# arihantb2/direct_lidar_odometry

Hardware: NVIDIA B200
Metric: scan_pairs_per_s (higher is better)
Workload: dtype f32 kNN / f64 GICP

## Files before the change

### direct_lidar_odometry_b200/csrc/knn_cov.cu

```cuda
#include <cstdio>
#include <cstdlib>
#include <mutex>
#include "internal.h"
#include "grid_search.cuh"
#include "gicp_math.cuh"
#include "sort_networks.inc"

namespace ngicp {

constexpr int KC_THREADS = 256;
constexpr int KC_WARPS = KC_THREADS / 32;
#ifndef KNN_MIN_BLOCKS
#define KNN_MIN_BLOCKS 5
#endif

__global__ void __launch_bounds__(KC_THREADS) knn_query_kernel(GridView g, const float4* __restrict__ queries, int nq, int k,
                                                               int* __restrict__ idx, float* __restrict__ d2) {
  const int lane = threadIdx.x & 31;
  const int warp = (blockIdx.x * blockDim.x + threadIdx.x) >> 5;
  const int nwarps = (gridDim.x * blockDim.x) >> 5;
  const GridParams gp = load_grid(g.desc);
  for (int q = warp; q < nq; q += nwarps) {
    const float4 qp = queries[q];
    WarpTopK rs;
// ... 6 lines not shown
      idx[(size_t)q * k + lane] = o;
      d2[(size_t)q * k + lane] = dd;
    }
  }
}

__global__ void __launch_bounds__(KC_THREADS, KNN_MIN_BLOCKS) knn_lists_kernel(GridView g, int n, int k, int* __restrict__ nbr, int q_lo, int q_hi) {
  const int lane = threadIdx.x & 31;
  const int warp = (blockIdx.x * blockDim.x + threadIdx.x) >> 5;
  const int nwarps = (gridDim.x * blockDim.x) >> 5;
  const GridParams gp = load_grid(g.desc);
  for (int q = q_lo + warp; q < q_hi; q += nwarps) {
    const float4 qp = __ldg(g.sorted + q);
    WarpTopK rs;
    rs.init(k, lane);
    if (isfinite(qp.x) && isfinite(qp.y) && isfinite(qp.z)) grid_search_warp(g, gp, qp.x, qp.y, qp.z, FLT_MAX, rs, k >= 4);
    if (lane < k) nbr[(size_t)q * k + lane] = rs.p;
  }
}

__global__ void __launch_bounds__(KC_THREADS) knn_query_wide_kernel(GridView g, const float4* __restrict__ queries, int nq, int k,
                                                                    int* __restrict__ idx, float* __restrict__ d2) {
  __shared__ float s_d[KC_WARPS][KNN_WIDE_MAX_K];
  __shared__ int s_p[KC_WARPS][KNN_WIDE_MAX_K];
  const int lane = threadIdx.x & 31, wib = threadIdx.x >> 5;
  const int warp = (blockIdx.x * blockDim.x + threadIdx.x) >> 5;
  const int nwarps = (gridDim.x * blockDim.x) >> 5;
  const GridParams gp = load_grid(g.desc);
  for (int q = warp; q < nq; q += nwarps) {
    const float4 qp = queries[q];
    WarpTopKWide rs;
    rs.init(k, lane, s_d[wib], s_p[wib]);
    if (isfinite(qp.x) && isfinite(qp.y) && isfinite(qp.z)) grid_search_warp(g, gp, qp.x, qp.y, qp.z, FLT_MAX, rs);
    __syncwarp();
    for (int j = lane; j < k; j += 32) {
      const int p = s_p[wib][j];
      idx[(size_t)q * k + j] = p >= 0 ? __float_as_int(__ldg(g.sorted + p).w) : -1;
      d2[(size_t)q * k + j] = p >= 0 ? s_d[wib][j] : -1.f;
    }
  }
}
__global__ void __launch_bounds__(KC_THREADS) knn_lists_wide_kernel(GridView g, int n, int k, int* __restrict__ nbr, int q_lo, int q_hi) {
  __shared__ float s_d[KC_WARPS][KNN_WIDE_MAX_K];
  __shared__ int s_p[KC_WARPS][KNN_WIDE_MAX_K];
  const int lane = threadIdx.x & 31, wib = threadIdx.x >> 5;
  const int warp = (blockIdx.x * blockDim.x + threadIdx.x) >> 5;
  const int nwarps = (gridDim.x * blockDim.x) >> 5;
  const GridParams gp = load_grid(g.desc);
  for (int q = q_lo + warp; q < q_hi; q += nwarps) {
    const float4 qp = __ldg(g.sorted + q);
    WarpTopKWide rs;
    rs.init(k, lane, s_d[wib], s_p[wib]);
    if (isfinite(qp.x) && isfinite(qp.y) && isfinite(qp.z)) grid_search_warp<WarpTopKWide, false, 4>(g, gp, qp.x, qp.y, qp.z, FLT_MAX, rs, true);
    __syncwarp();
    for (int j = lane; j < k; j += 32) nbr[(size_t)q * k + j] = s_p[wib][j];
  }
}

#ifndef TQ_WARPS
#define TQ_WARPS 2
#endif
#define TQ_POS_BITS 9
#define TQ_POS_MASK 0x1ffu
#ifndef TQ_CMAX
#define TQ_CMAX 448
#endif
#ifndef TQ_LCAP
#define TQ_LCAP 40
#endif
#ifndef TQ_CORE
#define TQ_CORE KNN_BRICK
#endif
#ifndef TQ_PACKED
#define TQ_PACKED 1
#endif
#ifndef TQ_UNROLL
#define TQ_UNROLL 1
#endif
#define NG_PRAGMA_(x) _Pragma(#x)
#define NG_UNROLL(n) NG_PRAGMA_(unroll n)
#ifndef TQ_SMAX
#define TQ_SMAX 16
#endif
constexpr int TQ_ITEM = 64;
struct TileSmem {
  float xs[TQ_CMAX], ys[TQ_CMAX], zs[TQ_CMAX];
  int slot[TQ_CMAX];
  unsigned lst[TQ_LCAP + 1][32];
  int cur[TQ_ITEM];
  float cur_t[TQ_ITEM];
  float cur_lo[TQ_ITEM], cur_hi[TQ_ITEM];
  int nxt[TQ_ITEM];
  int rowoff[68];
};

__device__ __forceinline__ float box_face_distance(const GridParams& gp, int x0, int x1, int y0, int y1, int z0, int z1,
                                                   float qx, float qy, float qz) {
  float m = FLT_MAX;
  if (x0 > 0) m = fminf(m, qx - (gp.ox + (float)x0 * gp.cell));
  if (x1 + 1 < gp.dx) m = fminf(m, (gp.ox + (float)(x1 + 1) * gp.cell) - qx);
  if (y0 > 0) m = fminf(m, qy - (gp.oy + (float)y0 * gp.cell));
  if (y1 + 1 < gp.dy) m = fminf(m, (gp.oy + (float)(y1 + 1) * gp.cell) - qy);
  if (z0 > 0) m = fminf(m, qz - (gp.oz + (float)z0 * gp.cell));
  if (z1 + 1 < gp.dz) m = fminf(m, (gp.oz + (float)(z1 + 1) * gp.cell) - qz);
  return m == FLT_MAX ? FLT_MAX : m - gp.margin;
}

#ifdef TQ_DEBUG
#define TQ_CHECK(cond, what, a, b) do { if (!(cond)) { printf("TQ_CHECK %s failed: %d %d (block %d thread %d)\n", what, (int)(a), (int)(b), blockIdx.x, threadIdx.x); __trap(); } } while (0)
#else
#define TQ_CHECK(cond, what, a, b) do { } while (0)
#endif
enum { ST_FALLBACK = 0, ST_TIES, ST_TILES, ST_PASSES, ST_LANES, ST_ITEMS, ST_DEC1, ST_DEC2, ST_DECHI, ST_PASS1, ST_PASS2, ST_PASSHI, ST_CAND, ST_TSUM, ST_TEND, ST_TSTART, ST_TWARPS, ST_N };
enum { CT_ITEMS = 0, CT_NEXT, CT_REST, CT_REST_NEXT, CT_DONE, CT_FIX, CT_SLOW, CT_N = 8 };

__device__ __forceinline__ void fb_append(unsigned mask, int slot, int lane, int* __restrict__ fb_list, int* __restrict__ fb_count,
                                          unsigned char* __restrict__ fb_flags) {
  if (!mask) return;
  if ((mask >> lane) & 1u) fb_flags[slot] = 1;
  const int leader = __ffs(mask) - 1;
  int base = 0;
  if (lane == leader) base = atomicAdd(fb_count, __popc(mask));
  base = __shfl_sync(FULL, base, leader);
  if ((mask >> lane) & 1u) fb_list[base + __popc(mask & ((1u << lane) - 1u))] = slot;
}

__device__ __forceinline__ void fix_append(unsigned mask, int slot, int lane, int n, int* __restrict__ fb_list, int* __restrict__ fix_count,
                                           unsigned char* __restrict__ fb_flags) {
  if (!mask) return;
  if ((mask >> lane) & 1u) fb_flags[slot] = 1;
  const int leader = __ffs(mask) - 1;
  int base = 0;
  if (lane == leader) base = atomicAdd(fix_count, __popc(mask));
  base = __shfl_sync(FULL, base, leader);
  if ((mask >> lane) & 1u) fb_list[n - 1 - (base + __popc(mask & ((1u << lane) - 1u)))] = slot;
}

__device__ __forceinline__ int warp_incl_scan(int v, int lane) {
#pragma unroll
  for (int o = 1; o < 32; o <<= 1) { const int t = __shfl_up_sync(FULL, v, o); if (lane >= o) v += t; }
  return v;
}
__device__ __forceinline__ int run_of(int inc, int t) {
  int j = 0;
#pragma unroll
  for (int step = 16; step > 0; step >>= 1) {
    const int v = __shfl_sync(FULL, inc, j + step - 1);
    if (v <= t) j += step;
  }
  return j;
}

__device__ __forceinline__ int box_population(const GridView& g, const GridParams& gp, int x0, int y0, int z0, int sz, int s, int sub, int nsub) {
  const int ny = sz + 2 * s, nrows = ny * ny;
  const int xl = max(x0 - s, 0), xr = min(x0 + sz - 1 + s, gp.dx - 1) + 1;
  int c = 0;
  for (int r = sub; r < nrows; r += nsub) {
    const int y = y0 - s + (r % ny), z = z0 - s + (r / ny);
    if (y >= 0 && y < gp.dy && z >= 0 && z < gp.dz && xl < xr) {
      const int* row = g.cell_start + (z * gp.dy + y) * gp.dx;
      c += __ldg(row + xr) - __ldg(row + xl);
    }
  }
  for (int o = nsub >> 1; o > 0; o >>= 1) c += __shfl_xor_sync(FULL, c, o);
  return c;
}

#ifndef TQ_BIG
#define TQ_BIG 32
#endif
__device__ __forceinline__ void emit_items(bool emit, bool slow, int x0, int y0, int z0, int sz, int q, int lane, int n, int4* __restrict__ items,
                                           int* __restrict__ ctrl) {
  const int nit = emit ? (q + TQ_ITEM - 1) / TQ_ITEM : 0;
  const int nfront = (slow || nit == 0 || q - (nit - 1) * TQ_ITEM > TQ_BIG) ? nit : nit - 1;
  const int nback = nit - nfront;
  if (__any_sync(FULL, nfront > 0)) {
    const int inc = warp_incl_scan(nfront, lane);
    const int total = __shfl_sync(FULL, inc, 31);
    int base = 0;
    if (lane == 0) base = atomicAdd(ctrl + CT_SLOW, total);
    base = __shfl_sync(FULL, base, 0) + inc - nfront;
    for (int i = 0; i < nfront; ++i) items[base + i] = make_int4(x0, y0, z0, sz | (i << 8));
  }
  const unsigned bm = __ballot_sync(FULL, nback > 0);
  if (bm) {
    int base = 0;
    if (lane == 0) base = atomicAdd(ctrl + CT_ITEMS, __popc(bm));
    base = __shfl_sync(FULL, base, 0) + __popc(bm & ((1u << lane) - 1u));
    if (nback > 0) items[n - 1 - base] = make_int4(x0, y0, z0, sz | ((nit - 1) << 8));
  }
}

__global__ void __launch_bounds__(256) brick_clear_kernel(GridView g, unsigned char* __restrict__ flags, long long flag_cap) {
  const GridParams gp = load_grid(g.desc);
  const long long nb = (long long)((gp.dx + TQ_CORE - 1) / TQ_CORE) * ((gp.dy + TQ_CORE - 1) / TQ_CORE) * ((gp.dz + TQ_CORE - 1) / TQ_CORE);
  if (nb > flag_cap) return;
// ... 11 lines not shown
  const int nbx = (gp.dx + TQ_CORE - 1) / TQ_CORE, nby = (gp.dy + TQ_CORE - 1) / TQ_CORE, nbz = (gp.dz + TQ_CORE - 1) / TQ_CORE;
  if ((long long)nbx * nby * nbz > flag_cap) return;
  for (int i = blockIdx.x * blockDim.x + threadIdx.x; i < n; i += gridDim.x * blockDim.x) {
    const float4 p = __ldg(g.sorted + i);
    const int bx = cell_coord(p.x, gp.ox, gp.inv, gp.dx) / TQ_CORE, by = cell_coord(p.y, gp.oy, gp.inv, gp.dy) / TQ_CORE,
              bz = cell_coord(p.z, gp.oz, gp.inv, gp.dz) / TQ_CORE;
    flags[((long long)bz * nby + by) * nbx + bx] = 1;
  }
}

#ifndef TQ_SLOW_FACTOR
#define TQ_SLOW_FACTOR 2
#endif
__global__ void __launch_bounds__(256) knn_plan_kernel(GridView g, int n, int k, int4* __restrict__ items, int* __restrict__ ctrl,
                                                       const unsigned char* __restrict__ flags, long long flag_cap) {
  const int lane = threadIdx.x & 31;
  const int nwarps = (gridDim.x * blockDim.x) >> 5;
  const GridParams gp = load_grid(g.desc);
  const int nbx = (gp.dx + TQ_CORE - 1) / TQ_CORE, nby = (gp.dy + TQ_CORE - 1) / TQ_CORE, nbz = (gp.dz + TQ_CORE - 1) / TQ_CORE;
  const int run = ((long long)nbx * nby * nbz > 32768) ? 8 : 1;
  const int nrx = (nbx + run - 1) / run;
  const int nruns = nrx * nby * nbz;
  for (int w = (blockIdx.x * blockDim.x + threadIdx.x) >> 5; w < nruns; w += nwarps) {
    const int rbx = (w % nrx) * run, rby = (w / nrx) % nby, rbz = w / (nrx * nby);
    unsigned occ = FULL;
    if (run > 1 && (long long)nbx * nby * nbz <= flag_cap) {
      int e = 0;
      if (lane < run && rbx + lane < nbx) e = flags[((long long)rbz * nby + rby) * nbx + rbx + lane];
      occ = __ballot_sync(FULL, e != 0);
      if (occ == 0u) continue;
    } else if (run > 1) {
      int e = 0;
      if (lane < TQ_CORE * TQ_CORE) {
        const int y = rby * TQ_CORE + (lane % TQ_CORE), z = rbz * TQ_CORE + (lane / TQ_CORE);
        if (y < gp.dy && z < gp.dz) {
          const int* row = g.cell_start + (z * gp.dy + y) * gp.dx;
          e = __ldg(row + min((rbx + run) * TQ_CORE, gp.dx)) - __ldg(row + rbx * TQ_CORE);
        }
      }
      if (!__any_sync(FULL, e != 0)) continue;
    }
    const int y0 = rby * TQ_CORE, z0 = rbz * TQ_CORE;
    unsigned deep_boxes;
    {
      const int bi = lane >> 2, sub = lane & 3;
      const bool valid = bi < run && rbx + bi < nbx && ((occ >> bi) & 1u);
      const int bx0 = valid ? (rbx + bi) * TQ_CORE : -(1 << 20);
      const int Qb = box_population(g, gp, bx0, y0, z0, TQ_CORE, 0, sub, 4);
      const int Cb = box_population(g, gp, Qb > 0 ? bx0 : -(1 << 20), y0, z0, TQ_CORE, 1, sub, 4);
      const bool fits = Qb > 0 && Cb <= TQ_CMAX;
      emit_items(sub == 0 && fits, Cb < TQ_SLOW_FACTOR * k, bx0, y0, z0, TQ_CORE, Qb, lane, n, items, ctrl);
      deep_boxes = __ballot_sync(FULL, sub == 0 && Qb > 0 && !fits);
    }
    for (; deep_boxes; deep_boxes &= deep_boxes - 1) {
      const int bi = (__ffs(deep_boxes) - 1) >> 2;
      const int x0 = (rbx + bi) * TQ_CORE;
      const int h = TQ_CORE / 2;
      const int ch = lane >> 2, sub = lane & 3;
      const int cx0 = x0 + (ch & 1) * h, cy0 = y0 + ((ch >> 1) & 1) * h, cz0 = z0 + (ch >> 2) * h;
      const int Qc = box_population(g, gp, cx0, cy0, cz0, h, 0, sub, 4);
      const int Cc = box_population(g, gp, cx0, cy0, cz0, h, 1, sub, 4);
      const bool fits = Cc <= TQ_CMAX;
      emit_items(sub == 0 && Qc > 0 && fits, false, cx0, cy0, cz0, h, Qc, lane, n, items, ctrl);
      unsigned deep = __ballot_sync(FULL, sub == 0 && Qc > 0 && !fits);
      for (; deep; deep &= deep - 1) {
        const int l = __ffs(deep) - 1;
        const int px = __shfl_sync(FULL, cx0, l), py = __shfl_sync(FULL, cy0, l), pz = __shfl_sync(FULL, cz0, l);
        const int gx = px + (ch & 1), gy = py + ((ch >> 1) & 1), gz = pz + (ch >> 2);
        const int Qg = box_population(g, gp, gx, gy, gz, 1, 0, sub, 4);
        emit_items(sub == 0 && Qg > 0, false, gx, gy, gz, 1, Qg, lane, n, items, ctrl);
      }
    }
  }
}

#ifndef TQ_TARGET_EXTRA
#define TQ_TARGET_EXTRA 14
#endif
__device__ __forceinline__ float lattice_floor(float t) { return __uint_as_float(__float_as_uint(t) & ~TQ_POS_MASK); }
struct Shrunk { float T2; int cnt; };
#ifndef TQ_SHRINK_F
#define TQ_SHRINK_F 0.75f
#endif
#ifndef TQ_COOP_SHRINK
#define TQ_COOP_SHRINK 1
#endif
#if TQ_COOP_SHRINK
__device__ __noinline__ Shrunk shrink_lists(TileSmem& S, unsigned om, float T2, int cnt) {
  const int lane = threadIdx.x & 31;
  const unsigned lt = (1u << lane) - 1u;
  Shrunk r;
  r.T2 = T2; r.cnt = cnt;
  for (; om; om &= om - 1) {
    const int L = __ffs(om) - 1;
    float t = __shfl_sync(FULL, T2, L);
    int n = __shfl_sync(FULL, cnt, L);
    do {
      t = lattice_floor(t * TQ_SHRINK_F);
      const unsigned tb = __float_as_uint(t);
      const unsigned e0 = lane < n ? S.lst[lane][L] : 0xffffffffu;
      const unsigned e1 = lane + 32 < n ? S.lst[lane + 32][L] : 0xffffffffu;
      const bool k0 = e0 < tb, k1 = e1 < tb;
      const unsigned m0 = __ballot_sync(FULL, k0), m1 = __ballot_sync(FULL, k1);
      __syncwarp();
      if (k0) S.lst[__popc(m0 & lt)][L] = e0;
      if (k1) S.lst[__popc(m0) + __popc(m1 & lt)][L] = e1;
      __syncwarp();
      n = __popc(m0) + __popc(m1);
    } while (n > TQ_LCAP - 4);
    if (lane == L) { r.T2 = t; r.cnt = n; }
  }
  return r;
}
#else
__device__ __noinline__ Shrunk shrink_list(unsigned* col, float T2, int cnt) {
  do {
    T2 = lattice_floor(T2 * 0.75f);
    const unsigned tb = __float_as_uint(T2);
    int pos = 0;
    for (int i = 0; i < cnt; ++i) {
      const unsigned e = col[i * 32];
      if (e < tb) { col[pos * 32] = e; ++pos; }
    }
    cnt = pos;
  } while (cnt > TQ_LCAP - 4);
  Shrunk r;
  r.T2 = T2; r.cnt = cnt;
  return r;
}
#endif
__device__ __forceinline__ unsigned long long f2_pack(float lo, float hi) { unsigned long long r; asm("mov.b64 %0, {%1, %2};" : "=l"(r) : "f"(lo), "f"(hi)); return r; }
__device__ __forceinline__ void f2_unpack(unsigned long long v, float& lo, float& hi) { asm("mov.b64 {%0, %1}, %2;" : "=f"(lo), "=f"(hi) : "l"(v)); }
__device__ __forceinline__ unsigned long long f2_sub(unsigned long long a, unsigned long long b) { unsigned long long r; asm("sub.rn.f32x2 %0, %1, %2;" : "=l"(r) : "l"(a), "l"(b)); return r; }
__device__ __forceinline__ unsigned long long f2_mul(unsigned long long a, unsigned long long b) { unsigned long long r; asm("mul.rn.f32x2 %0, %1, %2;" : "=l"(r) : "l"(a), "l"(b)); return r; }
__device__ __forceinline__ unsigned long long f2_fma(unsigned long long a, unsigned long long b, unsigned long long c) { unsigned long long r; asm("fma.rn.f32x2 %0, %1, %2, %3;" : "=l"(r) : "l"(a), "l"(b), "l"(c)); return r; }
struct Query2 { unsigned long long x, y, z, one; };
__device__ __forceinline__ unsigned long long sqdist2_unfused(const Query2& q, unsigned long long px, unsigned long long py, unsigned long long pz) {
#if TQ_PACKED
  const unsigned long long dx = f2_sub(q.x, px), dy = f2_sub(q.y, py), dz = f2_sub(q.z, pz);
  return f2_fma(f2_fma(f2_mul(dx, dx), q.one, f2_mul(dy, dy)), q.one, f2_mul(dz, dz));
#else
  float qx, qy, qz, t, x0, x1, y0, y1, z0, z1;
  f2_unpack(q.x, qx, t); f2_unpack(q.y, qy, t); f2_unpack(q.z, qz, t);
  f2_unpack(px, x0, x1); f2_unpack(py, y0, y1); f2_unpack(pz, z0, z1);
  return f2_pack(sqdist_unfused(qx, qy, qz, x0, y0, z0), sqdist_unfused(qx, qy, qz, x1, y1, z1));
#endif
}

__device__ __forceinline__ int collect_pass(TileSmem& S, unsigned* const col, int c, int cend, float qx, float qy, float qz, float one, float& T2_io, int cnt) {
  float T2 = T2_io;
  Query2 q;
  q.x = f2_pack(qx, qx); q.y = f2_pack(qy, qy); q.z = f2_pack(qz, qz); q.one = f2_pack(one, one);
  const unsigned a0 = (unsigned)__cvta_generic_to_shared(col);
  unsigned p = a0 + (unsigned)cnt * 128u;
  const unsigned plim = a0 + (unsigned)(TQ_LCAP - 4) * 128u;
#define TQ_OFFER(D, CI)                                                                                      \
  {                                                                                                          \
    asm volatile("st.shared.u32 [%0], %1;" ::"r"(p), "r"((__float_as_uint(D) & ~TQ_POS_MASK) | (unsigned)(CI)) : "memory"); \
    if ((D) < T2) p += 128u;                                                                                 \
  }
#if TQ_COOP_SHRINK
#define TQ_MAYBE_SHRINK()                                                       \
  {                                                                             \
    const unsigned om_ = __ballot_sync(FULL, p > plim);                         \
    if (om_) {                                                                  \
      const Shrunk r = shrink_lists(S, om_, T2, (int)((p - a0) >> 7));          \
      T2 = r.T2;                                                                \
      p = a0 + (unsigned)r.cnt * 128u;                                          \
    }                                                                           \
  }
#else
#define TQ_MAYBE_SHRINK()                                                       \
  if (p > plim) {                                                               \
    const Shrunk r = shrink_list(col, T2, (int)((p - a0) >> 7));                \
    T2 = r.T2;                                                                  \
    p = a0 + (unsigned)r.cnt * 128u;                                            \
  }
#endif
#define TQ_PAIR(CI)                                                                                                     \
  {                                                                                                                     \
    const unsigned long long d01 = sqdist2_unfused(q, *reinterpret_cast<const unsigned long long*>(S.xs + (CI)),        \
                                                   *reinterpret_cast<const unsigned long long*>(S.ys + (CI)),           \
                                                   *reinterpret_cast<const unsigned long long*>(S.zs + (CI)));          \
    float da, db;                                                                                                       \
    f2_unpack(d01, da, db);                                                                                             \
    TQ_OFFER(da, (CI)) TQ_OFFER(db, (CI) + 1)                                                                           \
  }
  if ((c & 2) && c < cend) { TQ_PAIR(c) TQ_MAYBE_SHRINK() c += 2; }
NG_UNROLL(TQ_UNROLL)
  for (; c + 4 <= cend; c += 4) {
    const ulonglong2 X = *reinterpret_cast<const ulonglong2*>(S.xs + c);
    const ulonglong2 Y = *reinterpret_cast<const ulonglong2*>(S.ys + c);
    const ulonglong2 Z = *reinterpret_cast<const ulonglong2*>(S.zs + c);
    const unsigned long long d01 = sqdist2_unfused(q, X.x, Y.x, Z.x), d23 = sqdist2_unfused(q, X.y, Y.y, Z.y);
    float d0, d1, d2, d3;
    f2_unpack(d01, d0, d1);
    f2_unpack(d23, d2, d3);
    TQ_OFFER(d0, c) TQ_OFFER(d1, c + 1) TQ_OFFER(d2, c + 2) TQ_OFFER(d3, c + 3)
    TQ_MAYBE_SHRINK()
  }
  if (c < cend) { TQ_PAIR(c) TQ_MAYBE_SHRINK() }
#undef TQ_PAIR
#undef TQ_OFFER
#undef TQ_MAYBE_SHRINK
  T2_io = T2;
  return (int)((p - a0) >> 7);
}

__device__ __noinline__ uint2 pick_kth(const unsigned* v, int k) { return make_uint2(v[k - 1], v[k]); }

template <int KT>
__global__ void __launch_bounds__(TQ_WARPS * 32) knn_lists_tile_kernel(GridView g, int n, int k_rt, int* __restrict__ nbr,
                                                                        const int4* __restrict__ items, int* __restrict__ ctrl,
                                                                        int* __restrict__ fb_list, unsigned char* __restrict__ fb_flags,
                                                                        unsigned long long* __restrict__ stats,
                                                                        int q_lo, int q_hi, float one ) {
  extern __shared__ __align__(16) unsigned char tq_smem_raw[];
  const int k = KT > 0 ? KT : k_rt;
  TileSmem& S = reinterpret_cast<TileSmem*>(tq_smem_raw)[threadIdx.x >> 5];
  const int lane = threadIdx.x & 31;
  const unsigned lt = (1u << lane) - 1u;
  const GridParams gp = load_grid(g.desc);
  const int nslow = ctrl[CT_SLOW];
  const int nitems = nslow + ctrl[CT_ITEMS];
  unsigned st_fb = 0, st_ties = 0, st_tiles = 0, st_passes = 0, st_lanes = 0, st_items = 0;
#ifdef TQ_STATS_DETAIL
  unsigned st_dec[3] = {0, 0, 0}, st_pass[3] = {0, 0, 0};
  unsigned long long st_cand = 0;
  unsigned long long st_t0;
  asm volatile("mov.u64 %0, %%globaltimer;" : "=l"(st_t0));
#endif

  for (;;) {
    int w = 0;
    if (lane == 0) w = atomicAdd(ctrl + CT_NEXT, 1);
    w = __shfl_sync(FULL, w, 0);
    if (w >= nitems) break;
    st_items++;
    const int4 item = __ldg(items + (w < nslow ? w : n - 1 - (w - nslow)));
    TQ_CHECK(nitems <= n, "nitems", nitems, n);
    const int x0 = item.x, y0 = item.y, z0 = item.z, sz = item.w & 255, first = (item.w >> 8) * TQ_ITEM;
    int ncur = 0;
    {
      int qa = 0, qlen = 0;
      if (lane < sz * sz) {
        const int y = y0 + (lane % sz), z = z0 + (lane / sz);
        if (y < gp.dy && z < gp.dz && x0 < gp.dx) {
          const int* row = g.cell_start + (z * gp.dy + y) * gp.dx;
          qa = __ldg(row + x0);
          qlen = __ldg(row + min(x0 + sz, gp.dx)) - qa;
        }
      }
      const int qinc = warp_incl_scan(qlen, lane);
      const int Q = __shfl_sync(FULL, qinc, 31);
      const int qexcl = qinc - qlen;
      ncur = min(TQ_ITEM, Q - first);
      int nkept = 0;
      for (int t0 = 0; t0 < ncur; t0 += 32) {
        const int t = first + t0 + lane;
        const int j = run_of(qinc, t);
        const int ja = __shfl_sync(FULL, qa, j), je = __shfl_sync(FULL, qexcl, j);
        const int slot = ja + (t - je);
        const bool keep = t0 + lane < ncur && slot >= q_lo && slot < q_hi;
        const unsigned km = __ballot_sync(FULL, keep);
        if (keep) {
          const int pos = nkept + __popc(km & lt);
          S.cur[pos] = slot; S.cur_t[pos] = 0.f; S.cur_lo[pos] = 0.f; S.cur_hi[pos] = -1.f;
        }
        nkept += __popc(km);
      }
      ncur = nkept;
      __syncwarp();
    }
    for (int s = 1; s <= TQ_SMAX && ncur > 0; s *= 2) {
      const int ny = sz + 2 * s, nrows = ny * ny;
      const int xl = max(x0 - s, 0), xr = min(x0 + sz - 1 + s, gp.dx - 1) + 1;
      int C = 0;
      bool overflow = false;
      for (int r0 = 0; r0 < nrows; r0 += 32) {
        const int r = r0 + lane;
        int a = 0, b = 0;
        if (r < nrows) {
          const int y = y0 - s + (r % ny), z = z0 - s + (r / ny);
          if (y >= 0 && y < gp.dy && z >= 0 && z < gp.dz) {
            const int* row = g.cell_start + (z * gp.dy + y) * gp.dx;
            a = __ldg(row + xl); b = __ldg(row + xr);
          }
        }
        if (!__any_sync(FULL, b != a)) {
          if (s <= 2 && r < nrows) S.rowoff[r] = C;
          continue;
        }
        const int len = b - a, plen = (len + 1) & ~1;
        const int inc = warp_incl_scan(plen, lane);
        const int Cr = __shfl_sync(FULL, inc, 31);
        if (C + Cr > TQ_CMAX) { overflow = true; break; }
        const int excl = inc - plen;
        if (s <= 2 && r < nrows) S.rowoff[r] = C + excl;
        for (int t0 = 0; t0 < Cr; t0 += 32) {
          const int t = t0 + lane;
          const int j = run_of(inc, t);
          const int ja = __shfl_sync(FULL, a, j), je = __shfl_sync(FULL, excl, j), jl = __shfl_sync(FULL, len, j);
          if (t < Cr) {
            const int off = t - je;
            float4 c = make_float4(INFINITY, 0.f, 0.f, 0.f);
            int p = -1;
            if (off < jl) { p = ja + off; c = __ldg(g.sorted + p); }
            S.xs[C + t] = c.x; S.ys[C + t] = c.y; S.zs[C + t] = c.z; S.slot[C + t] = p;
          }
        }
        C += Cr;
      }
      if (overflow) break;
      if (C < k) continue;
      if (s <= 2 && lane == 0) S.rowoff[nrows] = C;
      __syncwarp();
      st_tiles++;
      const float guess0 = (float)(k + TQ_TARGET_EXTRA) * (float)(ny * ny) * gp.cell * gp.cell / (3.14159265f * (float)C);
      int nnxt = 0;
      float prevT = 0.f;
      for (int round = 0; round < 8 && ncur > 0; ++round) {
        int nre = 0;
        for (int t0 = 0; t0 < ncur; t0 += 32) {
          const int t = t0 + lane;
          const bool has = t < ncur;
          int slot = has ? S.cur[t] : -1;
          float T2 = has ? S.cur_t[t] : 0.f;
          float lo = has ? S.cur_lo[t] : 0.f, hi = has ? S.cur_hi[t] : -1.f;
          float4 qp = make_float4(0.f, 0.f, 0.f, 0.f);
          if (has) qp = __ldg(g.sorted + slot);
          const bool me = has && isfinite(qp.x) && isfinite(qp.y) && isfinite(qp.z);
          if (has && !me)
            for (int j = 0; j < k; ++j) nbr[(size_t)slot * k + j] = -1;
          int ylo = 0, yhi = ny - 1, zlo = 0, zhi = ny - 1;
          if (s <= 2) {
            const int yy = cell_coord(qp.y, gp.oy, gp.inv, gp.dy) - (y0 - s), zz = cell_coord(qp.z, gp.oz, gp.inv, gp.dz) - (z0 - s);
            ylo = max(__reduce_min_sync(FULL, me ? yy : ny) - s, 0);
            yhi = min(__reduce_max_sync(FULL, me ? yy : -1) + s, ny - 1);
            zlo = max(__reduce_min_sync(FULL, me ? zz : ny) - s, 0);
            zhi = min(__reduce_max_sync(FULL, me ? zz : -1) + s, ny - 1);
          }
          float m2 = FLT_MAX;
          {
            const float m = box_face_distance(gp, x0 - s, x0 + sz - 1 + s, y0 - s + ylo, y0 - s + yhi, z0 - s + zlo, z0 - s + zhi, qp.x, qp.y, qp.z);
            if (m != FLT_MAX) m2 = m > 0.f ? m * m * 0.999999f : 0.f;
            m2 = lattice_floor(m2);
          }
          if (!(T2 > 0.f)) T2 = prevT > 0.f ? prevT * (float)(k + TQ_TARGET_EXTRA) / (float)k : guess0;
          T2 = lattice_floor(fminf(T2, m2));
          const bool active = me && m2 > 0.f && T2 > 0.f;
          st_passes++;
          st_lanes += __popc(__ballot_sync(FULL, active));
#ifdef TQ_STATS_DETAIL
          st_pass[s == 1 ? 0 : (s == 2 ? 1 : 2)]++;
          if (stats != nullptr) st_cand += s <= 2 ? (unsigned)max(S.rowoff[zhi * ny + yhi + 1] - S.rowoff[zlo * ny + ylo], 0) : (unsigned)C;
#endif
          int c_now = 0;
          const float T2_asked = T2;
          {
            float Tc = active ? T2 : -1.f;
            if (s <= 2) {
              for (int zr = zlo; zr <= zhi && yhi >= ylo; ++zr)
                c_now = collect_pass(S, &S.lst[0][lane], S.rowoff[zr * ny + ylo], S.rowoff[zr * ny + yhi + 1], qp.x, qp.y, qp.z, one, Tc, c_now);
            } else {
              c_now = collect_pass(S, &S.lst[0][lane], 0, C, qp.x, qp.y, qp.z, one, Tc, 0);
            }
            if (active) T2 = Tc;
          }
          const bool good = active && c_now >= k && c_now <= TQ_LCAP;
          const bool grow = me && (!active || (c_now < k && T2 >= m2));
          const bool retry = active && !good && !grow;
          bool decided = good;
          bool tie = false;
          bool needs_fix = false;
          float kth = T2;
          {
            const bool searching = good && (KT > 0 || c_now > k);
            const bool any_search = __any_sync(FULL, searching);
            if (any_search) {
              static_assert(TQ_LCAP == 40 || TQ_LCAP == 32, "the selection networks are generated for 32 and 40 wires");
              unsigned v[TQ_LCAP];
#pragma unroll
              for (int i = 0; i < TQ_LCAP; ++i) v[i] = (searching && i < c_now) ? S.lst[i][lane] : 0xffffffffu;
#define NG_UCAS(A, B) { const unsigned lo_ = min(v[A], v[B]), hi_ = max(v[A], v[B]); v[A] = lo_; v[B] = hi_; }
#if TQ_LCAP == 40
              NGICP_SORTNET_40(NG_UCAS)
#else
              NGICP_SORTNET_32(NG_UCAS)
#endif
#undef NG_UCAS
              unsigned vk, vk1;
              if (KT > 0) { vk = v[KT > 0 ? KT - 1 : 0]; vk1 = v[KT > 0 ? KT : 0]; }
              else { const uint2 pk = pick_kth(v, k); vk = pk.x; vk1 = pk.y; }
              unsigned bound = 0u;
              if (searching) {
                if ((vk >> TQ_POS_BITS) == (vk1 >> TQ_POS_BITS)) { tie = true; decided = false; st_ties++; }
                else { bound = ((vk >> TQ_POS_BITS) + 1u) << TQ_POS_BITS; kth = __uint_as_float(vk & ~TQ_POS_MASK); }
              }
              if (KT > 0) {
                bool near = false;
                constexpr int KW = KT > 0 ? KT : 4;
                int o[KW];
#pragma unroll
                for (int i = 0; i < KW; ++i) {
                  o[i] = S.slot[v[i] & TQ_POS_MASK];
                  if (i > 0) near = near || ((v[i - 1] >> TQ_POS_BITS) == (v[i] >> TQ_POS_BITS));
                }
                needs_fix = searching && !tie && near;
                if (searching && !tie) {
                  int* row = nbr + (size_t)slot * KW;
                  if (KW % 4 == 0) {
#pragma unroll
                    for (int i = 0; i < KW / 4; ++i) reinterpret_cast<int4*>(row)[i] = make_int4(o[4 * i], o[4 * i + 1], o[4 * i + 2], o[4 * i + 3]);
                  } else if (KW % 2 == 0) {
#pragma unroll
                    for (int i = 0; i < KW / 2; ++i) reinterpret_cast<int2*>(row)[i] = make_int2(o[2 * i], o[2 * i + 1]);
                  } else {
#pragma unroll
                    for (int i = 0; i < KW; ++i) row[i] = o[i];
                  }
                }
              } else {
                const bool compact = searching && !tie;
                int pos = 0;
#pragma unroll
                for (int i = 0; i < TQ_LCAP; ++i) {
                  const unsigned e = S.lst[i][lane];
                  if (compact && i < c_now && e < bound) { S.lst[pos][lane] = e; ++pos; }
                }
              }
            }
          }
          if (decided) prevT = kth;
          const unsigned dmask = __ballot_sync(FULL, decided);
#ifdef TQ_STATS_DETAIL
          st_dec[s == 1 ? 0 : (s == 2 ? 1 : 2)] += __popc(dmask);
#endif
          __syncwarp();
          for (unsigned mm = KT > 0 ? 0u : dmask; mm; mm &= mm - 1) {
            const int l = __ffs(mm) - 1;
            const int sl = __shfl_sync(FULL, slot, l);
            TQ_CHECK(lane >= k || ((S.lst[lane][l] & TQ_POS_MASK) < (unsigned)C && S.slot[S.lst[lane][l] & TQ_POS_MASK] >= 0), "tilepos", (int)(S.lst[lane][l] & TQ_POS_MASK), C);
            if (lane < k) nbr[(size_t)sl * k + lane] = S.slot[S.lst[lane][l] & TQ_POS_MASK];
          }
          __syncwarp();
          fix_append(__ballot_sync(FULL, needs_fix), slot, lane, n, fb_list, ctrl + CT_FIX, fb_flags);
          const unsigned tm = __ballot_sync(FULL, tie);
          st_fb += __popc(tm);
          fb_append(tm, slot, lane, fb_list, ctrl + CT_REST, fb_flags);
          const unsigned gm = __ballot_sync(FULL, grow);
          if (grow) S.nxt[nnxt + __popc(gm & lt)] = slot;
          nnxt += __popc(gm);
          const unsigned rm = __ballot_sync(FULL, retry);
          if (retry) {
            if (c_now < k) { lo = T2; if (T2 < T2_asked) hi = hi > 0.f ? fminf(hi, T2_asked) : T2_asked; } else hi = T2;
            float Tn = T2 * (float)(k + TQ_TARGET_EXTRA) / (float)max(c_now, 2);
            if (Tn <= lo || (hi > 0.f && Tn >= hi)) Tn = hi > 0.f ? 0.5f * (lo + hi) : T2 * 2.f;
            Tn = lattice_floor(fminf(Tn, m2));
            const int pos = nre + __popc(rm & lt);
            S.cur[pos] = slot;
            S.cur_t[pos] = Tn;
            S.cur_lo[pos] = lo;
            S.cur_hi[pos] = hi;
          }
          nre += __popc(rm);
          __syncwarp();
        }
        ncur = nre;
      }
      for (int t0 = 0; t0 < ncur; t0 += 32) {
        const bool has = t0 + lane < ncur;
        const int slot = has ? S.cur[t0 + lane] : -1;
        const unsigned m = __ballot_sync(FULL, has);
        if (has) S.nxt[nnxt + __popc(m & lt)] = slot;
        nnxt += __popc(m);
      }
      __syncwarp();
      for (int t = lane; t < nnxt; t += 32) { S.cur[t] = S.nxt[t]; S.cur_t[t] = 0.f; S.cur_lo[t] = 0.f; S.cur_hi[t] = -1.f; }
      ncur = nnxt;
      __syncwarp();
    }
    for (int t0 = 0; t0 < ncur; t0 += 32) {
      const bool has = t0 + lane < ncur;
      const int slot = has ? S.cur[t0 + lane] : -1;
      const unsigned m = __ballot_sync(FULL, has);
      st_fb += __popc(m);
      fb_append(m, slot, lane, fb_list, ctrl + CT_REST, fb_flags);
    }
    __syncwarp();
  }
  if (stats != nullptr && lane == 0) {
    atomicAdd(stats + ST_FALLBACK, (unsigned long long)st_fb);
    atomicAdd(stats + ST_TIES, (unsigned long long)st_ties);
    atomicAdd(stats + ST_TILES, (unsigned long long)st_tiles);
    atomicAdd(stats + ST_PASSES, (unsigned long long)st_passes);
    atomicAdd(stats + ST_LANES, (unsigned long long)st_lanes);
    atomicAdd(stats + ST_ITEMS, (unsigned long long)st_items);
#ifdef TQ_STATS_DETAIL
    atomicAdd(stats + ST_DEC1, (unsigned long long)st_dec[0]); atomicAdd(stats + ST_DEC2, (unsigned long long)st_dec[1]);
    atomicAdd(stats + ST_DECHI, (unsigned long long)st_dec[2]);
    atomicAdd(stats + ST_PASS1, (unsigned long long)st_pass[0]); atomicAdd(stats + ST_PASS2, (unsigned long long)st_pass[1]);
    atomicAdd(stats + ST_PASSHI, (unsigned long long)st_pass[2]);
    atomicAdd(stats + ST_CAND, st_cand);
    unsigned long long st_t1;
    asm volatile("mov.u64 %0, %%globaltimer;" : "=l"(st_t1));
    atomicAdd(stats + ST_TSUM, st_t1 - st_t0);
    atomicMax(stats + ST_TEND, st_t1);
    atomicMin(stats + ST_TSTART, st_t0);
    atomicAdd(stats + ST_TWARPS, 1ull);
#endif
  }
}

__global__ void __launch_bounds__(64) knn_lists_rest_kernel(GridView g, int k, int* __restrict__ nbr, const int* __restrict__ ctrl,
                                                                                     const int* __restrict__ fb_list) {
  const int lane = threadIdx.x & 31;
  const int warp = (blockIdx.x * blockDim.x + threadIdx.x) >> 5;
  const int nwarps = (gridDim.x * blockDim.x) >> 5;
  const GridParams gp = load_grid(g.desc);
  const int total = ctrl[CT_REST];
  for (int i = warp; i < total; i += nwarps) {
    const int q = fb_list[i];
    const float4 qp = __ldg(g.sorted + q);
    WarpTopK rs;
    rs.init(k, lane);
    if (isfinite(qp.x) && isfinite(qp.y) && isfinite(qp.z)) grid_search_warp<WarpTopK, false, 4>(g, gp, qp.x, qp.y, qp.z, FLT_MAX, rs, k >= 4);
    if (lane < k) nbr[(size_t)q * k + lane] = rs.p;
  }
}

template <int KT, bool SORTED>
__device__ __forceinline__ void cov_point(const GridView& g, int n, int k_rt, int method, const int* __restrict__ nbr, double* __restrict__ covs6,
                                          int q, int* __restrict__ idx_out, float* __restrict__ d2_out) {
  constexpr int KA = KT > 0 ? KT : (KT == 0 ? KNN_MAX_K : KNN_WIDE_MAX_K);
  const int k = KT > 0 ? KT : k_rt;
  const int* my = nbr + (size_t)q * k;
  const float4 qp = __ldg(g.sorted + q);
  const int orig = __float_as_int(qp.w);
  int ord[KA];
  if (KT > 0 && SORTED) {
#pragma unroll
    for (int j = 0; j < KA; ++j) ord[j] = __ldg(my + j);
  } else if (KT > 0) {
    unsigned long long key[KA];
    bool in_order = true;
#pragma unroll
    for (int j = 0; j < KA; ++j) {
      const int p = __ldg(my + j);
      TQ_CHECK(p < n, "nbr", p, q);
      key[j] = 0xffffffff00000000ull | (unsigned)j;
      if (p >= 0) {
        const float4 c = __ldg(g.sorted + p);
        key[j] = ((unsigned long long)__float_as_uint(sqdist_unfused(qp.x, qp.y, qp.z, c.x, c.y, c.z)) << 32) | (unsigned)p;
      }
      if (j > 0) in_order = in_order && key[j - 1] <= key[j];
    }
    if (!in_order) {
#define NG_CAS(A, B) { const unsigned long long ka = key[A], kb = key[B]; const bool sw = kb < ka; key[A] = sw ? kb : ka; key[B] = sw ? ka : kb; }
      if (KT == 10) { NGICP_SORTNET_10(NG_CAS) }
      else { NGICP_SORTNET_20(NG_CAS) }
#undef NG_CAS
    }
#pragma unroll
    for (int j = 0; j < KA; ++j) ord[j] = (key[j] >> 32) == 0xffffffffull ? -1 : (int)(unsigned)key[j];
  } else {
    unsigned long long key[KA];
    for (int j = 0; j < k; ++j) {
      const int p = __ldg(my + j);
      key[j] = 0xffffffff00000000ull | (unsigned)j;
      if (p >= 0) {
        const float4 c = __ldg(g.sorted + p);
        key[j] = ((unsigned long long)__float_as_uint(sqdist_unfused(qp.x, qp.y, qp.z, c.x, c.y, c.z)) << 32) | (unsigned)p;
      }
    }
    for (int j = 0; j < k; ++j) {
      int r = 0;
      for (int i = 0; i < k; ++i) r += key[i] < key[j] ? 1 : 0;
      ord[r] = __ldg(my + j);
    }
  }
  if (idx_out != nullptr) {
    for (int r = 0; r < k; ++r) {
      const int p = ord[r];
      int oi = -1;
      float dd = -1.f;
      if (p >= 0) { const float4 c = __ldg(g.sorted + p); oi = __float_as_int(c.w); dd = sqdist_unfused(qp.x, qp.y, qp.z, c.x, c.y, c.z); }
      idx_out[(size_t)orig * k + r] = oi;
      d2_out[(size_t)orig * k + r] = dd;
    }
    return;
  }
  double mx = 0.0, my_ = 0.0, mz = 0.0;
// ... 132 lines not shown
    static int sm_count[64] = {};
    const size_t smem = sizeof(TileSmem) * TQ_WARPS;
    int dev = 0;
    cudaGetDevice(&dev);
    const int di = dev & 63;
    {
      std::lock_guard<std::mutex> lock(attr_mutex);
      if (!attr_set[di]) {
        cudaError_t e = cudaFuncSetAttribute(knn_lists_tile_kernel<0>, cudaFuncAttributeMaxDynamicSharedMemorySize, (int)smem);
        if (e != cudaSuccess) return e;
        if ((e = cudaFuncSetAttribute(knn_lists_tile_kernel<10>, cudaFuncAttributeMaxDynamicSharedMemorySize, (int)smem)) != cudaSuccess) return e;
        if ((e = cudaFuncSetAttribute(knn_lists_tile_kernel<20>, cudaFuncAttributeMaxDynamicSharedMemorySize, (int)smem)) != cudaSuccess) return e;
        int occ[3] = {0, 0, 0};
        if ((e = cudaOccupancyMaxActiveBlocksPerMultiprocessor(&occ[0], knn_lists_tile_kernel<0>, TQ_WARPS * 32, smem)) != cudaSuccess) return e;
        if ((e = cudaOccupancyMaxActiveBlocksPerMultiprocessor(&occ[1], knn_lists_tile_kernel<10>, TQ_WARPS * 32, smem)) != cudaSuccess) return e;
        if ((e = cudaOccupancyMaxActiveBlocksPerMultiprocessor(&occ[2], knn_lists_tile_kernel<20>, TQ_WARPS * 32, smem)) != cudaSuccess) return e;
        blocks_per_sm[di] = occ[0] < occ[1] ? (occ[0] < occ[2] ? occ[0] : occ[2]) : (occ[1] < occ[2] ? occ[1] : occ[2]);
        if ((e = cudaDeviceGetAttribute(&sm_count[di], cudaDevAttrMultiProcessorCount, dev)) != cudaSuccess) return e;
        if (blocks_per_sm[di] < 1) blocks_per_sm[di] = 1;
        attr_set[di] = true;
      }
    }
    int* ctrl = nbr_scratch + (size_t)c.n * k;
    int* fb_list = ctrl + CT_N;
    int4* items = reinterpret_cast<int4*>(nbr_scratch + items_offset_ints(c.n, k));
    items = reinterpret_cast<int4*>((reinterpret_cast<uintptr_t>(items) + 15) & ~(uintptr_t)15);
    unsigned char* fb_flags = reinterpret_cast<unsigned char*>(nbr_scratch + flags_offset_ints(c.n, k));
    cudaError_t e = cudaSuccess;
    knn_zero_kernel<<<148, 256, 0, st>>>(ctrl, reinterpret_cast<unsigned*>(fb_flags), (c.n + 3) / 4);
    note_launches(1);
    unsigned long long* stats = nullptr;
    if (want_stats) {
      if (cudaMalloc(&stats, ST_N * sizeof(unsigned long long)) != cudaSuccess) return cudaGetLastError();
      cudaMemsetAsync(stats, 0, ST_N * sizeof(unsigned long long), st);
      cudaMemsetAsync(stats + ST_TSTART, 0xff, sizeof(unsigned long long), st);
    }
    const long long max_boxes = ((long long)table_cap + 63) / 64;
    long long plan_warps = max_boxes > 32768 ? (max_boxes + 7) / 8 + 1024 : max_boxes + 1024;
    unsigned char* bricks = reinterpret_cast<unsigned char*>(nbr_scratch + brick_offset_ints(c.n, k));
    const long long brick_cap = brick_flag_bytes(table_cap);
    if (c.bricks.p && c.bricks.bytes >= (size_t)brick_cap) {
      bricks = c.bricks.as<unsigned char>();
    } else {
      brick_clear_kernel<<<148 * 2, 256, 0, st>>>(c.view(), bricks, brick_cap);
      brick_mark_kernel<<<(c.n + 1023) / 1024, 256, 0, st>>>(c.view(), c.n, bricks, brick_cap);
      note_launches(2);
    }
    knn_plan_kernel<<<(unsigned)((plan_warps + 7) / 8), 256, 0, st>>>(c.view(), c.n, k, items, ctrl, bricks, brick_cap);
    note_launches(1);
    int tblocks = sm_count[di] * blocks_per_sm[di];
    const int tneed = (nq + 16 * TQ_WARPS - 1) / (16 * TQ_WARPS);
    if (tblocks > tneed) tblocks = tneed;
    const dim3 tgrid(tblocks), tblock(TQ_WARPS * 32);
    if (k == 10) knn_lists_tile_kernel<10><<<tgrid, tblock, smem, st>>>(c.view(), c.n, k, nbr_scratch, items, ctrl, fb_list, fb_flags, stats, q_lo, q_hi, 1.0f);
    else if (k == 20) knn_lists_tile_kernel<20><<<tgrid, tblock, smem, st>>>(c.view(), c.n, k, nbr_scratch, items, ctrl, fb_list, fb_flags, stats, q_lo, q_hi, 1.0f);
    else knn_lists_tile_kernel<0><<<tgrid, tblock, smem, st>>>(c.view(), c.n, k, nbr_scratch, items, ctrl, fb_list, fb_flags, stats, q_lo, q_hi, 1.0f);
    note_launches(2);
    const bool overlap = side != nullptr && side->stream != nullptr && !want_stats;
    cudaStream_t rs = overlap ? side->stream : st;
    if (overlap) {
      if ((e = cudaEventRecord(side->fork, st)) != cudaSuccess) return e;
      if ((e = cudaStreamWaitEvent(rs, side->fork, 0)) != cudaSuccess) return e;
    }
    knn_lists_rest_kernel<<<sm_count[di] * 16, 64, 0, rs>>>
       (c.view(), k, nbr_scratch, ctrl, fb_list);
    note_launches(1);
    launch_cov_rest_kernel(c, k, method, nbr_scratch, covs6, ctrl, fb_list, sm_count[di], rs);
    if (overlap && (e = cudaEventRecord(side->join, rs)) != cudaSuccess) return e;
    if (want_stats) {
      unsigned long long h[ST_N] = {};
      cudaMemcpyAsync(h, stats, sizeof(h), cudaMemcpyDeviceToHost, st);
      cudaStreamSynchronize(st);
      cudaFree(stats);
      fprintf(stderr, "[ngicp knn] n=%d k=%d warp-search=%llu (%.1f%%, ties %llu) items=%llu tiles=%llu passes=%llu lanes/pass=%.1f\n",
              c.n, k, h[ST_FALLBACK], 100.0 * (double)h[ST_FALLBACK] / (double)c.n, h[ST_TIES], h[ST_ITEMS], h[ST_TILES], h[ST_PASSES],
              h[ST_PASSES] ? (double)h[ST_LANES] / (double)h[ST_PASSES] : 0.0);
      fprintf(stderr, "[ngicp knn]   decided at radius 1 / 2 / >2: %llu / %llu / %llu, passes %llu / %llu / %llu, candidates per pass %.0f\n",
              h[ST_DEC1], h[ST_DEC2], h[ST_DECHI], h[ST_PASS1], h[ST_PASS2], h[ST_PASSHI],
              h[ST_PASSES] ? (double)h[ST_CAND] / (double)h[ST_PASSES] : 0.0);
      if (h[ST_TWARPS])
        fprintf(stderr, "[ngicp knn]   tile kernel: %llu warps, span %.1f us, mean warp busy %.1f us (%.0f%% of the span)\n", h[ST_TWARPS],
                1e-3 * (double)(h[ST_TEND] - h[ST_TSTART]), 1e-3 * (double)h[ST_TSUM] / (double)h[ST_TWARPS],
                100.0 * (double)h[ST_TSUM] / (double)h[ST_TWARPS] / (double)(h[ST_TEND] - h[ST_TSTART]));
    }
    launch_cov_kernel(c, k, method, nbr_scratch, covs6, q_lo, q_hi, fb_flags, nullptr, nullptr, st, k == 10 || k == 20);
    if (overlap && (e = cudaStreamWaitEvent(st, side->join, 0)) != cudaSuccess) return e;
    return cudaGetLastError();
  }
  launch_cov_kernel(c, k, method, nbr_scratch, covs6, q_lo, q_hi, nullptr, nullptr, nullptr, st);
  return cudaGetLastError();
}

}
```

Before: 1408.

## Refill retry lanes from a per-warp queue instead of round-based compaction in tile kNN

Replaces the round-based retry loop in the tile kNN kernel with a persistent-lane work queue. Each lane keeps retrying its own query, lanes that finish pull the next slot from shared memory, and queries that need a larger tile or exceed the retry limit are written back in place. This removes the cur/cur_t/cur_lo/cur_hi shared arrays and the partially filled rounds. It also widens the candidate vote to eight points per shrink check, which raises the list headroom reserve, and adds a minimum-blocks launch bound of 8 that may force register spills. Stats-only timing of the staging phase is added as well.

Result: slower. 1358 (median of 6 runs) (-3.6%).

```diff
diff --git a/direct_lidar_odometry_b200/csrc/knn_cov.cu b/direct_lidar_odometry_b200/csrc/knn_cov.cu
--- a/direct_lidar_odometry_b200/csrc/knn_cov.cu
+++ b/direct_lidar_odometry_b200/csrc/knn_cov.cu
@@ -112,14 +112,13 @@
 #ifndef TQ_SMAX
 #define TQ_SMAX 16
 #endif
-constexpr int TQ_ITEM = 64;
+#ifndef TQ_ITEM
+#define TQ_ITEM 64
+#endif
 struct TileSmem {
   float xs[TQ_CMAX], ys[TQ_CMAX], zs[TQ_CMAX];
   int slot[TQ_CMAX];
   unsigned lst[TQ_LCAP + 1][32];
-  int cur[TQ_ITEM];
-  float cur_t[TQ_ITEM];
-  float cur_lo[TQ_ITEM], cur_hi[TQ_ITEM];
   int nxt[TQ_ITEM];
   int rowoff[68];
 };
@@ -141,7 +140,7 @@
 #else
 #define TQ_CHECK(cond, what, a, b) do { } while (0)
 #endif
-enum { ST_FALLBACK = 0, ST_TIES, ST_TILES, ST_PASSES, ST_LANES, ST_ITEMS, ST_DEC1, ST_DEC2, ST_DECHI, ST_PASS1, ST_PASS2, ST_PASSHI, ST_CAND, ST_TSUM, ST_TEND, ST_TSTART, ST_TWARPS, ST_N };
+enum { ST_FALLBACK = 0, ST_TIES, ST_TILES, ST_PASSES, ST_LANES, ST_ITEMS, ST_DEC1, ST_DEC2, ST_DECHI, ST_PASS1, ST_PASS2, ST_PASSHI, ST_CAND, ST_TSUM, ST_TEND, ST_TSTART, ST_TWARPS, ST_TSTAGE, ST_N };
 enum { CT_ITEMS = 0, CT_NEXT, CT_REST, CT_REST_NEXT, CT_DONE, CT_FIX, CT_SLOW, CT_N = 8 };
 
 __device__ __forceinline__ void fb_append(unsigned mask, int slot, int lane, int* __restrict__ fb_list, int* __restrict__ fb_count,
@@ -319,6 +318,9 @@
 #ifndef TQ_SHRINK_F
 #define TQ_SHRINK_F 0.75f
 #endif
+#ifndef TQ_VOTE
+#define TQ_VOTE 8
+#endif
 #ifndef TQ_COOP_SHRINK
 #define TQ_COOP_SHRINK 1
 #endif
@@ -344,7 +346,7 @@
       if (k1) S.lst[__popc(m0) + __popc(m1 & lt)][L] = e1;
       __syncwarp();
       n = __popc(m0) + __popc(m1);
-    } while (n > TQ_LCAP - 4);
+    } while (n > TQ_LCAP - TQ_VOTE);
     if (lane == L) { r.T2 = t; r.cnt = n; }
   }
   return r;
@@ -360,7 +362,7 @@
       if (e < tb) { col[pos * 32] = e; ++pos; }
     }
     cnt = pos;
-  } while (cnt > TQ_LCAP - 4);
+  } while (cnt > TQ_LCAP - TQ_VOTE);
   Shrunk r;
   r.T2 = T2; r.cnt = cnt;
   return r;
@@ -390,7 +392,7 @@
   q.x = f2_pack(qx, qx); q.y = f2_pack(qy, qy); q.z = f2_pack(qz, qz); q.one = f2_pack(one, one);
   const unsigned a0 = (unsigned)__cvta_generic_to_shared(col);
   unsigned p = a0 + (unsigned)cnt * 128u;
-  const unsigned plim = a0 + (unsigned)(TQ_LCAP - 4) * 128u;
+  const unsigned plim = a0 + (unsigned)(TQ_LCAP - TQ_VOTE) * 128u;
 #define TQ_OFFER(D, CI)                                                                                      \
   {                                                                                                          \
     asm volatile("st.shared.u32 [%0], %1;" ::"r"(p), "r"((__float_as_uint(D) & ~TQ_POS_MASK) | (unsigned)(CI)) : "memory"); \
@@ -423,20 +425,28 @@
     f2_unpack(d01, da, db);                                                                                             \
     TQ_OFFER(da, (CI)) TQ_OFFER(db, (CI) + 1)                                                                           \
   }
+#define TQ_QUAD(CI)                                                                                                     \
+  {                                                                                                                     \
+    const ulonglong2 X = *reinterpret_cast<const ulonglong2*>(S.xs + (CI));                                             \
+    const ulonglong2 Y = *reinterpret_cast<const ulonglong2*>(S.ys + (CI));                                             \
+    const ulonglong2 Z = *reinterpret_cast<const ulonglong2*>(S.zs + (CI));                                             \
+    const unsigned long long d01 = sqdist2_unfused(q, X.x, Y.x, Z.x), d23 = sqdist2_unfused(q, X.y, Y.y, Z.y);          \
+    float d0, d1, d2, d3;                                                                                               \
+    f2_unpack(d01, d0, d1);                                                                                             \
+    f2_unpack(d23, d2, d3);                                                                                             \
+    TQ_OFFER(d0, (CI)) TQ_OFFER(d1, (CI) + 1) TQ_OFFER(d2, (CI) + 2) TQ_OFFER(d3, (CI) + 3)                             \
+  }
+  static_assert(TQ_VOTE == 4 || TQ_VOTE == 8, "a vote covers one or two 128-bit groups");
   if ((c & 2) && c < cend) { TQ_PAIR(c) TQ_MAYBE_SHRINK() c += 2; }
 NG_UNROLL(TQ_UNROLL)
-  for (; c + 4 <= cend; c += 4) {
-    const ulonglong2 X = *reinterpret_cast<const ulonglong2*>(S.xs + c);
-    const ulonglong2 Y = *reinterpret_cast<const ulonglong2*>(S.ys + c);
-    const ulonglong2 Z = *reinterpret_cast<const ulonglong2*>(S.zs + c);
-    const unsigned long long d01 = sqdist2_unfused(q, X.x, Y.x, Z.x), d23 = sqdist2_unfused(q, X.y, Y.y, Z.y);
-    float d0, d1, d2, d3;
-    f2_unpack(d01, d0, d1);
-    f2_unpack(d23, d2, d3);
-    TQ_OFFER(d0, c) TQ_OFFER(d1, c + 1) TQ_OFFER(d2, c + 2) TQ_OFFER(d3, c + 3)
+  for (; c + TQ_VOTE <= cend; c += TQ_VOTE) {
+    TQ_QUAD(c)
+    if (TQ_VOTE == 8) TQ_QUAD(c + 4)
     TQ_MAYBE_SHRINK()
   }
+  if (TQ_VOTE == 8 && c + 4 <= cend) { TQ_QUAD(c) TQ_MAYBE_SHRINK() c += 4; }
   if (c < cend) { TQ_PAIR(c) TQ_MAYBE_SHRINK() }
+#undef TQ_QUAD
 #undef TQ_PAIR
 #undef TQ_OFFER
 #undef TQ_MAYBE_SHRINK
@@ -446,8 +456,11 @@
 
 __device__ __noinline__ uint2 pick_kth(const unsigned* v, int k) { return make_uint2(v[k - 1], v[k]); }
 
+#ifndef TQ_MINB
+#define TQ_MINB 8
+#endif
 template <int KT>
-__global__ void __launch_bounds__(TQ_WARPS * 32) knn_lists_tile_kernel(GridView g, int n, int k_rt, int* __restrict__ nbr,
+__global__ void __launch_bounds__(TQ_WARPS * 32, TQ_MINB) knn_lists_tile_kernel(GridView g, int n, int k_rt, int* __restrict__ nbr,
                                                                         const int4* __restrict__ items, int* __restrict__ ctrl,
                                                                         int* __restrict__ fb_list, unsigned char* __restrict__ fb_flags,
                                                                         unsigned long long* __restrict__ stats,
@@ -464,7 +477,7 @@
 #ifdef TQ_STATS_DETAIL
   unsigned st_dec[3] = {0, 0, 0}, st_pass[3] = {0, 0, 0};
   unsigned long long st_cand = 0;
-  unsigned long long st_t0;
+  unsigned long long st_t0, st_tstage = 0;
   asm volatile("mov.u64 %0, %%globaltimer;" : "=l"(st_t0));
 #endif
 
@@ -477,7 +490,7 @@
     const int4 item = __ldg(items + (w < nslow ? w : n - 1 - (w - nslow)));
     TQ_CHECK(nitems <= n, "nitems", nitems, n);
     const int x0 = item.x, y0 = item.y, z0 = item.z, sz = item.w & 255, first = (item.w >> 8) * TQ_ITEM;
-    int ncur = 0;
+    int nq = 0;
     {
       int qa = 0, qlen = 0;
       if (lane < sz * sz) {
@@ -491,29 +504,30 @@
       const int qinc = warp_incl_scan(qlen, lane);
       const int Q = __shfl_sync(FULL, qinc, 31);
       const int qexcl = qinc - qlen;
-      ncur = min(TQ_ITEM, Q - first);
+      const int nitem = min(TQ_ITEM, Q - first);
       int nkept = 0;
-      for (int t0 = 0; t0 < ncur; t0 += 32) {
+      for (int t0 = 0; t0 < nitem; t0 += 32) {
         const int t = first + t0 + lane;
         const int j = run_of(qinc, t);
         const int ja = __shfl_sync(FULL, qa, j), je = __shfl_sync(FULL, qexcl, j);
         const int slot = ja + (t - je);
-        const bool keep = t0 + lane < ncur && slot >= q_lo && slot < q_hi;
+        const bool keep = t0 + lane < nitem && slot >= q_lo && slot < q_hi;
         const unsigned km = __ballot_sync(FULL, keep);
-        if (keep) {
-          const int pos = nkept + __popc(km & lt);
-          S.cur[pos] = slot; S.cur_t[pos] = 0.f; S.cur_lo[pos] = 0.f; S.cur_hi[pos] = -1.f;
-        }
+        if (keep) S.nxt[nkept + __popc(km & lt)] = slot;
         nkept += __popc(km);
       }
-      ncur = nkept;
+      nq = nkept;
       __syncwarp();
     }
-    for (int s = 1; s <= TQ_SMAX && ncur > 0; s *= 2) {
+    for (int s = 1; s <= TQ_SMAX && nq > 0; s *= 2) {
       const int ny = sz + 2 * s, nrows = ny * ny;
       const int xl = max(x0 - s, 0), xr = min(x0 + sz - 1 + s, gp.dx - 1) + 1;
       int C = 0;
       bool overflow = false;
+#ifdef TQ_STATS_DETAIL
+      unsigned long long st_s0;
+      asm volatile("mov.u64 %0, %%globaltimer;" : "=l"(st_s0));
+#endif
       for (int r0 = 0; r0 < nrows; r0 += 32) {
         const int r = r0 + lane;
         int a = 0, b = 0;
@@ -548,22 +562,34 @@
         }
         C += Cr;
       }
+#ifdef TQ_STATS_DETAIL
+      {
+        unsigned long long st_s1;
+        asm volatile("mov.u64 %0, %%globaltimer;" : "=l"(st_s1));
+        st_tstage += st_s1 - st_s0;
+      }
+#endif
       if (overflow) break;
       if (C < k) continue;
       if (s <= 2 && lane == 0) S.rowoff[nrows] = C;
       __syncwarp();
       st_tiles++;
       const float guess0 = (float)(k + TQ_TARGET_EXTRA) * (float)(ny * ny) * gp.cell * gp.cell / (3.14159265f * (float)C);
-      int nnxt = 0;
       float prevT = 0.f;
-      for (int round = 0; round < 8 && ncur > 0; ++round) {
-        int nre = 0;
-        for (int t0 = 0; t0 < ncur; t0 += 32) {
-          const int t = t0 + lane;
-          const bool has = t < ncur;
-          int slot = has ? S.cur[t] : -1;
-          float T2 = has ? S.cur_t[t] : 0.f;
-          float lo = has ? S.cur_lo[t] : 0.f, hi = has ? S.cur_hi[t] : -1.f;
+      int rd = 0, wr = 0;
+      int slot = -1, tries = 0;
+      float Tq = 0.f, lo = 0.f, hi = -1.f;
+      for (;;) {
+        {
+          const unsigned fm = __ballot_sync(FULL, slot < 0);
+          const int pos = rd + __popc(fm & lt);
+          if (slot < 0 && pos < nq) { slot = S.nxt[pos]; Tq = 0.f; lo = 0.f; hi = -1.f; tries = 0; }
+          rd = min(rd + __popc(fm), nq);
+        }
+        const bool has = slot >= 0;
+        if (!__any_sync(FULL, has)) break;
+        {
+          float T2 = Tq;
           float4 qp = make_float4(0.f, 0.f, 0.f, 0.f);
           if (has) qp = __ldg(g.sorted + slot);
           const bool me = has && isfinite(qp.x) && isfinite(qp.y) && isfinite(qp.z);
@@ -685,41 +711,26 @@
           const unsigned tm = __ballot_sync(FULL, tie);
           st_fb += __popc(tm);
           fb_append(tm, slot, lane, fb_list, ctrl + CT_REST, fb_flags);
-          const unsigned gm = __ballot_sync(FULL, grow);
-          if (grow) S.nxt[nnxt + __popc(gm & lt)] = slot;
-          nnxt += __popc(gm);
-          const unsigned rm = __ballot_sync(FULL, retry);
+          bool up = grow;
           if (retry) {
             if (c_now < k) { lo = T2; if (T2 < T2_asked) hi = hi > 0.f ? fminf(hi, T2_asked) : T2_asked; } else hi = T2;
             float Tn = T2 * (float)(k + TQ_TARGET_EXTRA) / (float)max(c_now, 2);
             if (Tn <= lo || (hi > 0.f && Tn >= hi)) Tn = hi > 0.f ? 0.5f * (lo + hi) : T2 * 2.f;
-            Tn = lattice_floor(fminf(Tn, m2));
-            const int pos = nre + __popc(rm & lt);
-            S.cur[pos] = slot;
-            S.cur_t[pos] = Tn;
-            S.cur_lo[pos] = lo;
-            S.cur_hi[pos] = hi;
+            Tq = lattice_floor(fminf(Tn, m2));
+            up = ++tries >= 8;
           }
-          nre += __popc(rm);
+          const unsigned gm = __ballot_sync(FULL, up);
+          if (up) S.nxt[wr + __popc(gm & lt)] = slot;
+          wr += __popc(gm);
+          if (!(retry && !up)) slot = -1;
           __syncwarp();
         }
-        ncur = nre;
       }
-      for (int t0 = 0; t0 < ncur; t0 += 32) {
-        const bool has = t0 + lane < ncur;
-        const int slot = has ? S.cur[t0 + lane] : -1;
-        const unsigned m = __ballot_sync(FULL, has);
-        if (has) S.nxt[nnxt + __popc(m & lt)] = slot;
-        nnxt += __popc(m);
-      }
-      __syncwarp();
-      for (int t = lane; t < nnxt; t += 32) { S.cur[t] = S.nxt[t]; S.cur_t[t] = 0.f; S.cur_lo[t] = 0.f; S.cur_hi[t] = -1.f; }
-      ncur = nnxt;
-      __syncwarp();
-    }
-    for (int t0 = 0; t0 < ncur; t0 += 32) {
-      const bool has = t0 + lane < ncur;
-      const int slot = has ? S.cur[t0 + lane] : -1;
+      nq = wr;
+    }
+    for (int t0 = 0; t0 < nq; t0 += 32) {
+      const bool has = t0 + lane < nq;
+      const int slot = has ? S.nxt[t0 + lane] : -1;
       const unsigned m = __ballot_sync(FULL, has);
       st_fb += __popc(m);
       fb_append(m, slot, lane, fb_list, ctrl + CT_REST, fb_flags);
@@ -745,6 +756,7 @@
     atomicMax(stats + ST_TEND, st_t1);
     atomicMin(stats + ST_TSTART, st_t0);
     atomicAdd(stats + ST_TWARPS, 1ull);
+    atomicAdd(stats + ST_TSTAGE, st_tstage);
 #endif
   }
 }
@@ -1043,6 +1055,9 @@
         fprintf(stderr, "[ngicp knn]   tile kernel: %llu warps, span %.1f us, mean warp busy %.1f us (%.0f%% of the span)\n", h[ST_TWARPS],
                 1e-3 * (double)(h[ST_TEND] - h[ST_TSTART]), 1e-3 * (double)h[ST_TSUM] / (double)h[ST_TWARPS],
                 100.0 * (double)h[ST_TSUM] / (double)h[ST_TWARPS] / (double)(h[ST_TEND] - h[ST_TSTART]));
+    if (h[ST_TSUM])
+      fprintf(stderr, "[ngicp knn]   staging %.1f us per warp (%.0f%% of the warps' busy time)\n",
+              1e-3 * (double)h[ST_TSTAGE] / (double)h[ST_TWARPS], 100.0 * (double)h[ST_TSTAGE] / (double)h[ST_TSUM]);
     }
     launch_cov_kernel(c, k, method, nbr_scratch, covs6, q_lo, q_hi, fb_flags, nullptr, nullptr, st, k == 10 || k == 20);
     if (overlap && (e = cudaStreamWaitEvent(st, side->join, 0)) != cudaSuccess) return e;
```
